# BarnitaSharma/Part-based-3D-Reconstruction

Measured on AMD Instinct MI355X. Metric: Mvoxel/s carved (semantic carve, 1024^3 grid), higher is better.
Workload: dtype u8

## Files before the change

part-based-3d-reconstruction_amd/csrc/ctx.hip:

```cpp
#include <cmath>
#include <cstdlib>

#include <string>

#include "pb3d_internal.h"

static int pool_flush(pb3d_ctx* ctx);

static thread_local char g_err[512] = "";

void pb3d_set_error(const char* fmt, ...) {
    va_list ap;
    va_start(ap, fmt);
    vsnprintf(g_err, sizeof(g_err), fmt, ap);
    va_end(ap);
}

extern "C" {

int pb3d_version(void) { return 101; }

int64_t pb3d_sync_count(pb3d_ctx* ctx) { return ctx ? (int64_t)ctx->sync_count : -1; }

const char* pb3d_last_error(void) { return g_err; }

int pb3d_device_count(int* n) {
    PB3D_REQUIRE(n != nullptr, "pb3d_device_count: null output");
    int c = 0;
    hipError_t e = hipGetDeviceCount(&c);
    if (e != hipSuccess) {
        (void)hipGetLastError();
        c = 0;
    }
    *n = c;
    return PB3D_OK;
}

int pb3d_create(int device, pb3d_ctx** out) {
    PB3D_REQUIRE(out != nullptr, "pb3d_create: null output");
    *out = nullptr;
    int n = 0;
    pb3d_device_count(&n);
    if (n <= 0) {
        pb3d_set_error("pb3d_create: no HIP device visible (libpb3d has no CPU fallback)");
        return PB3D_ENODEVICE;
    }
    PB3D_REQUIRE(device >= 0 && device < n, "pb3d_create: device %d out of range (have %d)", device, n);
    PB3D_HIP(hipSetDevice(device));
    pb3d_ctx* ctx = (pb3d_ctx*)calloc(1, sizeof(pb3d_ctx));
    if (!ctx) {
        pb3d_set_error("pb3d_create: out of host memory");
        return PB3D_ENOMEM;
    }
    ctx->device = device;
    {
        auto env_int = [](const char* name) { const char* v = getenv(name); return v ? atoi(v) : 0; };
        ctx->tune_uncap = env_int("PB3D_UNCAP");
        ctx->tune_sliced = env_int("PB3D_SLICED");
        ctx->tune_s32_gpw = env_int("PB3D_S32_GPW");
        ctx->tune_rot90_wide = env_int("PB3D_ROT90_WIDE");
    }
    hipDeviceProp_t prop;
    hipError_t e = hipGetDeviceProperties(&prop, device);
    if (e != hipSuccess) {
        free(ctx);
        pb3d_set_error("hipGetDeviceProperties failed: %s", hipGetErrorString(e));
        return PB3D_ENODEVICE;
    }
    ctx->cus = prop.multiProcessorCount;
    e = hipStreamCreateWithFlags(&ctx->stream, hipStreamNonBlocking);
    if (e != hipSuccess) {
        free(ctx);
        pb3d_set_error("hipStreamCreate failed: %s", hipGetErrorString(e));
        return PB3D_ENODEVICE;
    }
    e = hipEventCreateWithFlags(&ctx->s32_ev, hipEventDisableTiming);
    if (e != hipSuccess) {
        (void)hipStreamDestroy(ctx->stream);
        free(ctx);
        pb3d_set_error("hipEventCreate failed: %s", hipGetErrorString(e));
        return PB3D_ENODEVICE;
    }
    {
        const char* v = getenv("PB3D_DEVICE_POOL_MB");
        ctx->pool_cap = v ? (size_t)(atoll(v) < 0 ? 0 : atoll(v)) << 20 : (size_t)prop.totalGlobalMem / 4;
    }
    ctx->pinned_bytes = 1 << 16;
    e = hipHostMalloc(&ctx->pinned, ctx->pinned_bytes, hipHostMallocDefault);
    if (e != hipSuccess) {
        (void)hipEventDestroy(ctx->s32_ev);
        (void)hipStreamDestroy(ctx->stream);
        free(ctx);
        pb3d_set_error("hipHostMalloc failed: %s", hipGetErrorString(e));
        return PB3D_ENOMEM;
    }
    if (const char* kn = getenv("PB3D_KNOBS")) {
        std::string all(kn);
        size_t pos = 0;
        while (pos < all.size()) {
            const size_t end = all.find(',', pos);
            const std::string item = all.substr(pos, end == std::string::npos ? std::string::npos : end - pos);
            pos = end == std::string::npos ? all.size() : end + 1;
            if (item.empty()) continue;
            const size_t eq = item.find('=');
            const int rc = eq == std::string::npos ? PB3D_EINVAL : pb3d_set_tuning(ctx, item.substr(0, eq).c_str(), atoi(item.c_str() + eq + 1));
            if (rc != PB3D_OK) {
                if (eq == std::string::npos) pb3d_set_error("PB3D_KNOBS: '%s' is not name=value", item.c_str());
                (void)hipHostFree(ctx->pinned);
                (void)hipEventDestroy(ctx->s32_ev);
                (void)hipStreamDestroy(ctx->stream);
                free(ctx);
                return PB3D_EINVAL;
            }
        }
    }
    *out = ctx;
    return PB3D_OK;
}

namespace {
struct Knob { const char* name; int pb3d_ctx::*field; int lo, hi; const char* what; };
const Knob kKnobs[] = {
    {"sliced", &pb3d_ctx::tune_sliced, 0, 1, "0 (rotation steps on 0/1 data run bit-sliced) or 1 (never: byte chain)"},
    {"rot90_wide", &pb3d_ctx::tune_rot90_wide, 0, 2, "0 (choose), 1 or 2 (the 128-tile / 128-byte-segment kernels)"},
    {"rot90_fill", &pb3d_ctx::tune_rot90_fill, 0, 64, "a count of workgroups per CU (0 = the built-in rule)"},
    {"rot90_order", &pb3d_ctx::tune_rot90_order, 0, 1, "0 (a plane chunk per XCD) or 1 (plain x-fastest order)"},
    {"rot90_flat", &pb3d_ctx::tune_rot90_flat, 0, 2, "0 (choose), 1 (row-wise tile kernel) or 2 (flat on whole-line streams only)"},
    {"rot90_mask_block", &pb3d_ctx::tune_rot90_mask_block, 0, 1, "0 (mask bytes once into LDS) or 1 (per plane / segment)"},
    {"s32_gpw", &pb3d_ctx::tune_s32_gpw, 0, 1 << 20, "a count of plane groups"},
    {"s32_order", &pb3d_ctx::tune_s32_order, 0, 1, "0 (plane groups fastest) or 1 (x fastest)"},
    {"s32_fuse_last", &pb3d_ctx::tune_s32_fuse_last, 0, 1, "0 (fused) or 1 (table step)"},
    {"ccl_blocks", &pb3d_ctx::tune_ccl_blocks, 0, 1 << 20, "a count of workgroups per CU"},
    {"ccl_init_blocks", &pb3d_ctx::tune_ccl_init_blocks, 0, 1 << 20, "a count of workgroups per CU"},
    {"ccl_tilecols", &pb3d_ctx::tune_ccl_tilecols, 0, 64, "at most 64"},
    {"ccl_merge", &pb3d_ctx::tune_ccl_merge, 0, 1, "0 (tile kernels) or 1 (pairwise kernel)"},
    {"orient_tile", &pb3d_ctx::tune_orient_tile, 0, 1, "0 (128-pixel tiles where they apply) or 1 (never)"},
    {"global_composed", &pb3d_ctx::tune_global_composed, 0, 1, "0 (mask bits -> sliced chain -> colours) or 1 (ones -> process -> colour)"},
    {"per_job", &pb3d_ctx::tune_per_job, 0, 1, "0 (merged / fused forms) or 1 (job by job)"},
    {"no_table_cache", &pb3d_ctx::tune_no_table_cache, 0, 1, "0 (tables cached across calls) or 1 (rebuilt every call)"},
    {"part90_inflight", &pb3d_ctx::tune_part90_inflight, 0, 44, "10 UA + UE with UA, UE in 1, 2, 4 (0 = the default 2 / 4)"},
    {"crop_ablate", &pb3d_ctx::tune_crop_ablate, 0, 1 << 20, "ablation switches of k_crop_chain"},
    {"uncap", &pb3d_ctx::tune_uncap, 0, 1, "0 or 1 (every grid-stride kernel as one workgroup per tile)"},
};
}

int pb3d_set_tuning(pb3d_ctx* ctx, const char* name, int value) {
    PB3D_REQUIRE(ctx != nullptr && name != nullptr, "pb3d_set_tuning: null argument");
    for (const Knob& k : kKnobs)
        if (!strcmp(name, k.name)) {
            PB3D_REQUIRE(value >= k.lo && value <= k.hi, "pb3d_set_tuning: %s is %s (got %d)", k.name, k.what, value);
            ctx->*k.field = value;
            return PB3D_OK;
        }
    pb3d_set_error("pb3d_set_tuning: unknown knob '%s'", name);
    return PB3D_EINVAL;
}

int pb3d_make_current(pb3d_ctx* ctx) {
    PB3D_REQUIRE(ctx != nullptr, "pb3d_make_current: null context");
    PB3D_HIP(hipSetDevice(ctx->device));
    return PB3D_OK;
}

void pb3d_destroy(pb3d_ctx* ctx) {
    if (!ctx) return;
    (void)hipSetDevice(ctx->device);
    (void)hipStreamSynchronize(ctx->stream);
    pb3d_comm_destroy(ctx);
    (void)pool_flush(ctx);
    for (int i = 0; i < PB3D_SLOT_COUNT; ++i)
        if (ctx->scratch[i]) (void)hipFree(ctx->scratch[i]);
    if (ctx->pinned) (void)hipHostFree(ctx->pinned);
    if (ctx->stage) (void)hipHostFree(ctx->stage);
    (void)hipEventDestroy(ctx->s32_ev);
    (void)hipStreamDestroy(ctx->stream);
    free(ctx);
}

int pb3d_device_info(pb3d_ctx* ctx, char* name, int name_cap, int* compute_units, int64_t* hbm_bytes) {
    PB3D_REQUIRE(ctx != nullptr, "pb3d_device_info: null context");
    hipDeviceProp_t prop;
    PB3D_HIP(hipGetDeviceProperties(&prop, ctx->device));
    if (name && name_cap > 0) {
        snprintf(name, (size_t)name_cap, "%s (%s)", prop.name, prop.gcnArchName);
    }
    if (compute_units) *compute_units = prop.multiProcessorCount;
    if (hbm_bytes) *hbm_bytes = (int64_t)prop.totalGlobalMem;
    return PB3D_OK;
}

int pb3d_sync(pb3d_ctx* ctx) {
    PB3D_REQUIRE(ctx != nullptr, "pb3d_sync: null context");
    return pb3d_stream_sync(ctx);
}

static int pool_flush(pb3d_ctx* ctx) {
    if (ctx->pool_nfree == 0) return PB3D_OK;
    PB3D_HIP(hipStreamSynchronize(ctx->stream));
    for (int i = 0; i < ctx->pool_nfree; ++i) (void)hipFree(ctx->pool_free[i].p);
    ctx->pool_nfree = 0;
    ctx->pool_cached = 0;
    return PB3D_OK;
}

static hipError_t pool_malloc(pb3d_ctx* ctx, void** p, size_t bytes) {
    hipError_t e = hipMalloc(p, bytes);
    if (e == hipErrorOutOfMemory && ctx->pool_nfree > 0) {
        (void)hipGetLastError();
        if (pool_flush(ctx) == PB3D_OK) e = hipMalloc(p, bytes);
    }
    return e;
}

int pb3d_dev_alloc(pb3d_ctx* ctx, size_t bytes, void** dptr) {
    PB3D_REQUIRE(ctx != nullptr && dptr != nullptr, "pb3d_dev_alloc: null argument");
    *dptr = nullptr;
    PB3D_HIP(hipSetDevice(ctx->device));
    size_t padded = ((bytes ? bytes : 1) + 64 + 255) & ~(size_t)255;
    int best = -1;
    for (int i = 0; i < ctx->pool_nfree; ++i) {
        const size_t b = ctx->pool_free[i].bytes;
        if (b >= padded && b <= padded + padded / 8 + (1u << 20) && (best < 0 || b < ctx->pool_free[best].bytes)) best = i;
    }
    void* p = nullptr;
    size_t got = padded;
    if (best >= 0) {
        p = ctx->pool_free[best].p; got = ctx->pool_free[best].bytes;
        ctx->pool_cached -= got;
        ctx->pool_free[best] = ctx->pool_free[--ctx->pool_nfree];
    } else {
        PB3D_HIP(pool_malloc(ctx, &p, padded));
    }
    if (ctx->pool_cap > 0) {
        if (ctx->pool_nlive < PB3D_POOL_LIVE) ctx->pool_live[ctx->pool_nlive++] = {p, got, 0};
    }
    *dptr = p;
    return PB3D_OK;
}

int pb3d_dev_free(pb3d_ctx* ctx, void* dptr) {
    PB3D_REQUIRE(ctx != nullptr, "pb3d_dev_free: null context");
    if (!dptr) return PB3D_OK;
    size_t bytes = 0;
    for (int i = ctx->pool_nlive - 1; i >= 0; --i)
        if (ctx->pool_live[i].p == dptr) { bytes = ctx->pool_live[i].bytes; ctx->pool_live[i] = ctx->pool_live[--ctx->pool_nlive]; break; }
    if (bytes > 0 && bytes <= ctx->pool_cap) {
        while (ctx->pool_nfree > 0 && (ctx->pool_cached + bytes > ctx->pool_cap || ctx->pool_nfree == PB3D_POOL_SLOTS)) {
            int old = 0;
            for (int i = 1; i < ctx->pool_nfree; ++i)
                if (ctx->pool_free[i].stamp < ctx->pool_free[old].stamp) old = i;
            PB3D_TRY(pb3d_stream_sync(ctx));
            PB3D_HIP(hipFree(ctx->pool_free[old].p));
            ctx->pool_cached -= ctx->pool_free[old].bytes;
            ctx->pool_free[old] = ctx->pool_free[--ctx->pool_nfree];
        }
        ctx->pool_free[ctx->pool_nfree++] = {dptr, bytes, ++ctx->pool_stamp};
        ctx->pool_cached += bytes;
        return PB3D_OK;
    }
    PB3D_TRY(pb3d_stream_sync(ctx));
    PB3D_HIP(hipFree(dptr));
    return PB3D_OK;
}

int pb3d_dev_memset(pb3d_ctx* ctx, void* dptr, int value, size_t bytes) {
    PB3D_REQUIRE(ctx != nullptr && (dptr != nullptr || bytes == 0), "pb3d_dev_memset: null argument");
    if (bytes) PB3D_HIP(hipMemsetAsync(dptr, value, bytes, ctx->stream));
    return PB3D_OK;
}

int pb3d_h2d(pb3d_ctx* ctx, void* dptr, const void* hptr, size_t bytes) {
    PB3D_REQUIRE(ctx != nullptr, "pb3d_h2d: null context");
    if (!bytes) return PB3D_OK;
    PB3D_REQUIRE(dptr && hptr, "pb3d_h2d: null buffer");
    PB3D_HIP(hipMemcpyAsync(dptr, hptr, bytes, hipMemcpyHostToDevice, ctx->stream));
    return pb3d_stream_sync(ctx);
}

int pb3d_h2d_async(pb3d_ctx* ctx, void* dptr, const void* hptr, size_t bytes) {
    PB3D_REQUIRE(ctx != nullptr, "pb3d_h2d_async: null context");
    if (!bytes) return PB3D_OK;
    PB3D_REQUIRE(dptr && hptr, "pb3d_h2d_async: null buffer");
    if (!ctx->stage) {
// ... 137 lines not shown
```

part-based-3d-reconstruction_amd/csrc/pb3d_internal.h:

```cpp
#pragma once
#include <hip/hip_runtime.h>

#include <cstdarg>
#include <cstdint>
#include <cstdio>
#include <cstring>
#include <initializer_list>
#include <type_traits>

#include "pb3d.h"

typedef uint8_t u8;
typedef int64_t i64;
typedef uint64_t u64;
typedef uint32_t u32;

enum pb3d_slot : int {
    PB3D_SLOT_HOST_IN0 = 0,
    PB3D_SLOT_HOST_OUT0 = 1,
    PB3D_SLOT_HOST_IN1 = 2,
    PB3D_SLOT_HOST_OUT1 = PB3D_SLOT_HOST_IN1,
    PB3D_SLOT_HOST_IN2 = 3,
    PB3D_SLOT_HOST_OUT2 = PB3D_SLOT_HOST_IN2,
    PB3D_SLOT_HOST_TMP = PB3D_SLOT_HOST_IN2,
// ... 10 lines not shown
    PB3D_SLOT_RECOLOR_FLAGS = PB3D_SLOT_VOL_TMP,
    PB3D_SLOT_SELECT_FLAGS = PB3D_SLOT_VOL_KEEP,
    PB3D_SLOT_MESH_HOST_COLS = PB3D_SLOT_VOL_OCC,
    PB3D_SLOT_BLOCK_COUNTS = 8,
    PB3D_SLOT_SCAN_LOCAL = 11,
    PB3D_SLOT_SCAN_SEGS = 15,
    PB3D_SLOT_PROJ_WINNER = PB3D_SLOT_BLOCK_COUNTS,
    PB3D_SLOT_DEFORM_ACC = PB3D_SLOT_SCAN_LOCAL,
    PB3D_SLOT_POINTS_OFFSETS = 9,
    PB3D_SLOT_POINTS_MASKS = 25,
    PB3D_SLOT_EXTRACT_OFFSETS = 24,
    PB3D_SLOT_EXTRACT_MASKS = 26,
    PB3D_SLOT_DEFORM_MARKS = 12,
    PB3D_SLOT_DEFORM_BATCH_MARKS = PB3D_SLOT_DEFORM_MARKS,
    PB3D_SLOT_DEFORM_PTS = 13,
    PB3D_SLOT_DEFORM_COLS = 14,
    PB3D_SLOT_PROJ_BATCH_CAMS = 20,
    PB3D_SLOT_PROJ_BATCH_COUNTS = 21,
    PB3D_SLOT_PROJ_BATCH_COLORS = 22,
    PB3D_SLOT_DEFORM_BATCH_TUPLES = PB3D_SLOT_PROJ_BATCH_CAMS,
    PB3D_SLOT_DEFORM_BATCH_COUNTS = PB3D_SLOT_PROJ_BATCH_COUNTS,
    PB3D_SLOT_MEMBERS_COUNTS = 16,
    PB3D_SLOT_MEMBERS_OFFSETS = 17,
    PB3D_SLOT_LABEL_FLAG = 23,
    PB3D_SLOT_NN_REF_COUNTS = 18,
    PB3D_SLOT_NN_REF_STARTS = 19,
    PB3D_SLOT_NN_REF_COORDS = 27,
    PB3D_SLOT_NN_QUERY_COUNTS = 28,
    PB3D_SLOT_NN_QUERY_STARTS = 29,
    PB3D_SLOT_NN_ORDER = 30,
    PB3D_SLOT_NN_SCAN_LOCAL = 31,
    PB3D_SLOT_NN_SCAN_SEGS = 33,
    PB3D_SLOT_NN_BOUNDS_PARTIALS = 41,
    PB3D_SLOT_NN_BOUNDS = 47,
    PB3D_SLOT_VIOU_BITS = 44,
    PB3D_SLOT_VIOU_DILATED = 45,
    PB3D_SLOT_ROT_VALID_TABLE = 10,
    PB3D_SLOT_PART90_JOBS_T = 46,
    PB3D_SLOT_S32_TILE_PROGRAMS = 32,
    PB3D_SLOT_SLICED_FLAG = 34,
    PB3D_SLOT_SLICED_MASK_BITS = 35,
    PB3D_SLOT_GUIDED_DESCS = 36,
    PB3D_SLOT_GUIDED_MASKS = 37,
    PB3D_SLOT_GUIDED_TABLES = 38,
    PB3D_SLOT_GUIDED_COUNTS = 39,
    PB3D_SLOT_GUIDED_SLICES = 43,
    PB3D_SLOT_CCL_RECORDS = 40,
    PB3D_SLOT_CCL_MEMBER_BITS = 42,
    PB3D_SLOT_MESH_BITS = 48,
    PB3D_SLOT_MESH_VERT_OFFSETS = 51,
    PB3D_SLOT_MESH_FACE_OFFSETS = 52,
    PB3D_SLOT_MESH_VERT_COUNTS = 49,
    PB3D_SLOT_MESH_FACE_COUNTS = 50,
    PB3D_SLOT_MESH_VSCAN_LOCAL = 53,
    PB3D_SLOT_MESH_VSCAN_SEGS = 54,
    PB3D_SLOT_MESH_FSCAN_LOCAL = 55,
    PB3D_SLOT_MESH_FSCAN_SEGS = 56,
    PB3D_SLOT_MESH_VERT_BASE = 57,
    PB3D_SLOT_IOU_COUNTS = 58,
    PB3D_SLOT_KNN_REF_IDS = 59,
    PB3D_SLOT_SURF_FLAG = 60,
    PB3D_SLOT_SURF_FACE_NORMALS = 61,
    PB3D_SLOT_SURF_VERT_COUNTS = 62,
    PB3D_SLOT_SURF_VERT_STARTS = 63,
    PB3D_SLOT_SURF_INCIDENT = 64,
    PB3D_SLOT_SURF_SCAN_LOCAL = 65,
    PB3D_SLOT_SURF_SCAN_SEGS = 66,
    PB3D_SLOT_DENSITY_BOUNDS = 67,
    PB3D_SLOT_DENSITY_COUNTS = 68,
    PB3D_SLOT_DENSITY_WEIGHTS = 69,
    PB3D_SLOT_ICP_INDEX_STARTS = 70,
    PB3D_SLOT_ICP_INDEX_COORDS = 71,
    PB3D_SLOT_ICP_INDEX_IDS = 72,
    PB3D_SLOT_ICP_MOVED = 73,
    PB3D_SLOT_ICP_NEAREST = 74,
    PB3D_SLOT_ICP_PARTIALS = 75,
    PB3D_SLOT_PLANE_PARTIALS = 76,
    PB3D_SLOT_CROP_COUNTS = 77,
    PB3D_SLOT_CROP_OFFSETS = 78,
    PB3D_SLOT_CROP_SCAN_LOCAL = 79,
    PB3D_SLOT_CROP_SCAN_SEGS = 80,
    PB3D_SLOT_SELECT = 81,
    PB3D_SLOT_ICP_KEYS = 82,

    PB3D_SLOT_COUNT = 83
};

struct pb3d_nn_grid {
    double lo[3], hi[3];
    double inv[3], h[3];
    int n[3];
    i64 ncells;
};
struct pb3d_nn_index {
    pb3d_nn_grid g;
    i64 nr;
    const i64* starts;
    const double* xs;
    const int* ids;
};
constexpr i64 pb3d_max_points = (1ll << 31) - 1;
template <bool F64>
__device__ __forceinline__ void pb3d_load3(const void* p, i64 i, double* x, double* y, double* z) {
    if (F64) {
        const double* d = (const double*)p + 3 * i;
        *x = d[0]; *y = d[1]; *z = d[2];
    } else {
        const float* f = (const float*)p + 3 * i;
        *x = (double)f[0]; *y = (double)f[1]; *z = (double)f[2];
    }
}
template <bool F64>
__device__ __forceinline__ void pb3d_load3(const void* p, i64 i, double v[3]) { pb3d_load3<F64>(p, i, &v[0], &v[1], &v[2]); }

struct pb3d_pair {
    bool valid;
    int nslots;
    pb3d_slot slot[3];
    u64 use[3];
};

#define PB3D_POOL_SLOTS 64
#define PB3D_POOL_LIVE 4096

struct pb3d_event {
    hipEvent_t ev;
};

struct pb3d_ctx {
    int device;
    int cus;
    hipStream_t stream;
    bool orient_lds_set;
    bool guided_lds_set;
    int tune_rot90_fill;
    int tune_rot90_order;
    int tune_rot90_flat;
    int tune_rot90_mask_block;
    int tune_orient_tile;
    int tune_global_composed;
    int tune_per_job;
    int tune_no_table_cache;
    int tune_part90_inflight;
    int tune_crop_ablate;
    int tune_uncap;
    int tune_sliced;
    int tune_rot90_wide;
    bool rot90w_lds_set;
    bool part90_lds_set;
    bool rot90wf_lds_set;
    int tune_s32_order;
    int tune_s32_fuse_last;
    int tune_s32_gpw;
    int tune_ccl_blocks;
    int tune_ccl_init_blocks;
    int tune_ccl_tilecols;
    int tune_ccl_merge;
    void* scratch[PB3D_SLOT_COUNT];
    size_t scratch_bytes[PB3D_SLOT_COUNT];
    void* pinned;
    size_t pinned_bytes;
    void* stage;
    size_t stage_bytes, stage_head;
    u64 sync_count;
    struct PointsArgs { const void* grid; i64 A0, A1, A2, n, C, ncolors, stride; u8 colors[3 * 32]; };
    struct { pb3d_pair pair; PointsArgs a; } pts_dev, pts;
    struct MeshArgs { const void* grid; i64 A0, A1, A2, nv, nf, C, stride; };
    struct { pb3d_pair pair; MeshArgs a; } mesh_dev, mesh;
    struct { pb3d_pair pair; int ox, oy, oz; i64 X, Y, Z, n; } deform;
    struct ValidCache { void* buf; u64 gen; i64 W, D; double p[8]; } valid_cache;
    struct S32Cache { bool valid; u64 gen; i64 W, D; int ns; double p[32 * 8]; } s32_cache;
    hipEvent_t s32_ev;
    struct CclLast { bool valid; const void* labels; const void* bits; i64 rows, A2, P; u64 gen; bool members_only; int K, C; u32 colors[PB3D_CCL_MAX_COLORS]; } ccl_last;
    struct IcpIndex { bool valid; const void* tgt; i64 nt; int f64; u64 gen[3]; pb3d_nn_index ix; } icp_index;
    struct PoolBlock { void* p; size_t bytes; u64 stamp; };
    PoolBlock pool_free[PB3D_POOL_SLOTS];
    int pool_nfree;
    PoolBlock pool_live[PB3D_POOL_LIVE];
    int pool_nlive;
    size_t pool_cached, pool_cap;
    u64 pool_stamp;
    u64 scratch_gen;
    u64 scratch_slot_gen[PB3D_SLOT_COUNT];
    u64 scratch_use[PB3D_SLOT_COUNT];
    void* rccl_lib;
    void* rccl_comm;
    int rank, nranks;
};

void pb3d_set_error(const char* fmt, ...);

#define PB3D_HIP(call)                                                                          \
    do {                                                                                        \
        hipError_t e_ = (call);                                                                 \
        if (e_ != hipSuccess) {                                                                 \
            pb3d_set_error("%s failed: %s (%s:%d)", #call, hipGetErrorString(e_), __FILE__, __LINE__); \
            return e_ == hipErrorOutOfMemory ? PB3D_ENOMEM : PB3D_ENODEVICE;                    \
        }                                                                                       \
    } while (0)

#define PB3D_TRY(call)                 \
    do {                               \
        int rc_ = (call);              \
        if (rc_ != PB3D_OK) return rc_; \
    } while (0)

#define PB3D_REQUIRE(cond, ...)         \
    do {                                \
        if (!(cond)) {                  \
            pb3d_set_error(__VA_ARGS__); \
            return PB3D_EINVAL;         \
        }                               \
    } while (0)

#define PB3D_CHECK_LAUNCH() PB3D_HIP(hipGetLastError())

int pb3d_scratch(pb3d_ctx* ctx, pb3d_slot slot, size_t bytes, void** out);

void pb3d_pair_record(pb3d_ctx* ctx, pb3d_pair* pr, std::initializer_list<pb3d_slot> slots);
int pb3d_pair_check(const pb3d_ctx* ctx, const pb3d_pair& pr, bool same_args, const char* fill, const char* count);
template <class Args>
bool pb3d_same_args(const Args& a, const Args& b) {
    static_assert(std::has_unique_object_representations_v<Args>, "an argument record compared byte for byte must have no padding");
    return memcmp(&a, &b, sizeof(Args)) == 0;
}
static inline pb3d_ctx::PointsArgs pb3d_points_args(const void* grid, i64 A0, i64 A1, i64 A2, int C, const u8* colors, int ncolors,
                                                    int stride, i64 n) {
    pb3d_ctx::PointsArgs a{grid, A0, A1, A2, n, C, ncolors, stride, {}};
    if (ncolors) memcpy(a.colors, colors, (size_t)(C == 1 ? 1 : 3) * ncolors);
    return a;
}
int pb3d_stream_sync(pb3d_ctx* ctx);

static inline unsigned pb3d_stream_blocks(const pb3d_ctx* ctx, i64 work_items, int per_block, int blocks_per_cu) {
    i64 need = (work_items + per_block - 1) / per_block;
    i64 cap = (blocks_per_cu > 0 && !ctx->tune_uncap) ? (i64)(ctx->cus > 0 ? ctx->cus : 256) * blocks_per_cu : 0x7fffffffll;
    if (need < 1) need = 1;
    return (unsigned)(need < cap ? need : cap);
}

static inline unsigned pb3d_batch_blocks(const pb3d_ctx* ctx, i64 work_items, int per_block, i64 batch, int blocks_per_cu) {
    i64 need = (work_items + per_block - 1) / per_block;
    const i64 cap = ((i64)ctx->cus * blocks_per_cu + batch - 1) / batch;
    if (need > cap) need = cap;
    return (unsigned)(need < 1 ? 1 : need);
}

struct pb3d_magic { u32 m; int sa, sb; u32 d; };
static inline pb3d_magic pb3d_make_magic(u32 d) {
    int L = 0;
    while ((1ull << L) < d) ++L;
    pb3d_magic g;
    g.m = (u32)(((1ull << 32) * ((1ull << L) - d)) / d + 1);
    g.sa = L < 1 ? L : 1;
    g.sb = L > 1 ? L - 1 : 0;
    g.d = d;
    return g;
}
__device__ __forceinline__ u32 pb3d_div(u32 n, const pb3d_magic g) {
    const u32 t = __umulhi(g.m, n);
    return (t + ((n - t) >> g.sa)) >> g.sb;
}

struct pb3d_ccl_dev { const i64* total; const char* records; int dcap; };
int pb3d_ccl_label_on_device(pb3d_ctx* ctx, const uint8_t* d_grid, int64_t A0, int64_t A1, int64_t A2, const uint8_t color[3], int channels, int32_t* d_labels,
                             int64_t cap, pb3d_ccl_dev* dev, int connectivity = 6);

int pb3d_scan_counts(pb3d_ctx* ctx, const u32* d_counts, i64 n, i64* d_offsets, pb3d_slot local_slot, pb3d_slot seg_slot);
int pb3d_nn_index_build(pb3d_ctx* ctx, const void* d_r, int r_f64, i64 nr, pb3d_slot starts_slot, pb3d_slot coords_slot, pb3d_slot ids_slot,
                        pb3d_nn_index* ix);
int pb3d_nn_index_nearest(pb3d_ctx* ctx, const pb3d_nn_index& ix, const double* d_q, i64 nq, int* d_idx);
int pb3d_select_kth(pb3d_ctx* ctx, const double* d_vals, i64 n, const i64* d_rank, double* d_out);
int pb3d_process_grid_sliced(pb3d_ctx* ctx, const u8* d_occ, i64 W, i64 H, i64 D, const u8* d_mask_wh, int angle_interval, u8* d_out,
                             int known_binary, int* took);
int pb3d_global_carve_sliced(pb3d_ctx* ctx, const u8* d_mask_wh, const u8* d_rgb_hw3, i64 W, i64 H, i64 D, int angle_interval, u8* d_out_rgb,
                             int* took);
int pb3d_process_grid_binary_dev(pb3d_ctx* ctx, const u8* d_occ, i64 W, i64 H, i64 D, const u8* d_mask_wh, int angle_interval, u8* d_out,
                                 u8* d_tmp);
int pb3d_rotate_step_sliced(pb3d_ctx* ctx, const u8* d_occ, i64 W, i64 H, i64 D, const double M[9], const double off[3], const u8* d_mask_wh, u8* d_out,
                            int* took);
int pb3d_launch_rotate_generic(pb3d_ctx* ctx, const u8* d_in, i64 W, i64 H, i64 D, const double M[9],
                               const double off[3], const u8* d_mask_wh, u8* d_out, const u8* d_mask_src);
bool pb3d_is_perm_step(const double M[9], const double off[3], i64 W, i64 D);
int pb3d_perm_valid_table(pb3d_ctx* ctx, const double M[9], const double off[3], i64 W, i64 D, u32** bits, int* nw, int* c0, int* c2, bool* rot90);
bool pb3d_perm_step_ok(const double M[9], const double off[3], i64 W, i64 D, const void* a, const void* b);
int pb3d_launch_rotate_perm(pb3d_ctx* ctx, const u8* d_in, i64 W, i64 H, i64 D, const double M[9], const double off[3],
                            const u8* d_mask_src, const u8* d_mask_dst, u8* d_out);
int pb3d_try_part_carve90(pb3d_ctx* ctx, const u8* d_colored, int C, i64 W, i64 H, i64 D, const u8* d_mask_sub, const u8* d_mask_carve,
                          const int* job_angle, const int* job_skip, int njobs, u8* d_out);
int pb3d_transpose_mask_dev(pb3d_ctx* ctx, const u8* d_hw, i64 h, i64 w, u8* d_wh);
int pb3d_part_carve90_planes(pb3d_ctx* ctx, const u8* d_colored, int C, i64 W, i64 H, i64 D, const u32* d_A, const u32* d_AT, int njobs, const u32* d_vbits,
                             int nwv, int c0, int c2, u8* d_out, int* took);
int pb3d_launch_gc90_stream(pb3d_ctx* ctx, const u8* d_bin_hw, const u8* d_rgb_hw3, int C, const u32* d_vbits, int nw, int c0, i64 W, i64 H, i64 D, i64 x0,
                            i64 x1, u8* d_out_slab);
int pb3d_launch_global_carve90(pb3d_ctx* ctx, const u8* d_bin_hw, const u8* d_rgb_hw3, int C, i64 h, i64 w, const double M[9],
                               const double off[3], i64 x0, i64 x1, u8* d_out_slab);
```

part-based-3d-reconstruction_amd/csrc/sliced.hip:

```cpp
#include "rot_common.h"

namespace {

typedef u32 u32x4 __attribute__((ext_vector_type(4)));
typedef u32 u32x2 __attribute__((ext_vector_type(2)));
typedef u32x2 u32x2_a1 __attribute__((aligned(1)));

constexpr int ST = 64;
constexpr int STHREADS = 256;
constexpr int SROWS = 96;
#ifndef PB3D_SPITCH
#define PB3D_SPITCH 101
#endif
constexpr int SPITCH = PB3D_SPITCH;
constexpr int SMAXU = 9;
constexpr int SMAXSTEPS = 32;

struct STile {
    int bx0, bz0, nrows, nunits, fits, pad0, pad1, pad2;
    u32 ugoff[SMAXU * STHREADS];
    unsigned short uloff[SMAXU * STHREADS];
    u32 cellw[16 * STHREADS];
};
static_assert(sizeof(STile) % 16 == 0, "STile is read with 16-byte loads");
// ... 275 lines not shown
        const int idx = tid + 256 * k, r = idx >> 3, cg = idx & 7;
        u32* dst = tile + r * UPITCH + 4 * cg;
        dst[0] = dq[k].x; dst[1] = dq[k].y; dst[2] = dq[k].z; dst[3] = dq[k].w;
    }
    __syncthreads();
    const int zp = tid & 7, xl = tid >> 3;
    const i64 x = x0 + xl, z = z0 + 16 * zp;
    const bool rowlive = x < W;
    const bool live = rowlive && z < D;
    const u32 vb = live ? (vbits[x * nw + (z >> 5)] >> (z & 31)) & 0xffffu : 0u;
    const u32 m = rowlive ? mbits[(i64)g * W + x] : 0u;
    const int np = (int)(H - 32 * (i64)g < 32 ? H - 32 * (i64)g : 32);
    u32 v[4][4];
#pragma unroll
    for (int j = 0; j < 4; ++j) {
        u32 a[4];
#pragma unroll
        for (int c = 0; c < 4; ++c) a[c] = ((vb >> (4 * j + c)) & 1u) ? tile[(16 * zp + 4 * j + c) * UPITCH + xl] & m : 0u;
        tr4x4(a[0], a[1], a[2], a[3], v[j]);
    }
    const bool fullrow = z0 + UZ <= D;
    const i64 rowbase = (((i64)(rowlive ? x : 0) * H + 32 * (i64)g) * D + z0) * 3;
    const u8* px = rgb_hw3 + ((32 * (i64)g) * W + (rowlive ? x : 0)) * 3;
    const int grp = (lane & ~7) * 3;
#pragma unroll
    for (int q = 0; q < 32; ++q) {
        if (q >= np) continue;
        u32 o[12];
        {
            const u8* c = px + (i64)q * W * 3;
            const u32 R = c[0], G = c[1], B = c[2];
            const u32 C0 = R | (G << 8) | (B << 16) | (R << 24), C1 = G | (B << 8) | (R << 16) | (G << 24), C2 = B | (R << 8) | (G << 16) | (B << 24);
#pragma unroll
            for (int j = 0; j < 4; ++j) rgb4((v[j][q >> 3] >> (q & 7)) & 0x01010101u, C0, C1, C2, o + 3 * j);
        }
        if (!fullrow) {
            if (live) {
                u8* dp = out + rowbase + (i64)q * D * 3 + 48 * zp;
                for (int bb = 0; bb < 48 && 3 * z + bb < 3 * D; ++bb) dp[bb] = (u8)(o[bb >> 2] >> (8 * (bb & 3)));
            }
            continue;
        }
#pragma unroll
        for (int k = 0; k < 3; ++k) { u32x4 t4; t4.x = o[4 * k]; t4.y = o[4 * k + 1]; t4.z = o[4 * k + 2]; t4.w = o[4 * k + 3]; win[wv][3 * lane + k] = t4; }
#pragma unroll
        for (int k = 0; k < 3; ++k) {
            const int cidx = 8 * k + zp;
            const u32x4 t4 = win[wv][grp + cidx];
            if (rowlive) *(u32x4_a1*)(out + rowbase + (i64)q * D * 3 + 16 * cidx) = t4;
        }
    }
}

__global__ __launch_bounds__(STHREADS) void k_s32_prep(StepParams sp, i64 W, i64 D, i64 Dp, int ntz, STile* __restrict__ tiles) {
    __shared__ int bb[4];
    __shared__ int rmin[SROWS], rmax[SROWS];
    __shared__ int ustart[SROWS + 1];
    __shared__ int rc0[SROWS];
    const int tid = threadIdx.x;
    const RotParams p = sp.p[blockIdx.y];
    const int t = (int)blockIdx.x;
    STile* o = tiles + (i64)blockIdx.y * gridDim.x + t;
    const i64 x0 = (i64)(t / ntz) * ST, z0 = (i64)(t % ntz) * ST;
    if (tid == 0) { bb[0] = 0x7fffffff; bb[1] = -1; bb[2] = 0x7fffffff; bb[3] = -1; }
    if (tid < SROWS) { rmin[tid] = 0x7fffffff; rmax[tid] = -1; }
    __syncthreads();
    const int tz = tid & 15, jr = tid >> 4;
    int s0[16], s2[16];
    u32 lut[16];
    int mn0 = 0x7fffffff, mx0 = -1, mn2 = 0x7fffffff, mx2 = -1;
#pragma unroll
    for (int i = 0; i < 4; ++i)
#pragma unroll
        for (int c = 0; c < 4; ++c) {
            const int k = 4 * i + c;
            const i64 x = x0 + jr + 16 * i, z = z0 + 4 * tz + c;
            s0[k] = -1; s2[k] = 0; lut[k] = 0;
            if (x < W && z < D) {
                const Cell cl = make_cell(p, x, z, W, D);
                if (cl.s0 >= 0) {
                    s0[k] = cl.s0; s2[k] = cl.s2;
                    lut[k] = lut_of(cl) | (cl.wx1 != 0.0 ? 1u << 16 : 0u) | (cl.wz1 != 0.0 ? 1u << 17 : 0u);
                    const int e0 = cl.s0 + (int)((lut[k] >> 16) & 1u), e2 = cl.s2 + (int)((lut[k] >> 17) & 1u);
                    mn0 = min(mn0, cl.s0); mx0 = max(mx0, e0); mn2 = min(mn2, cl.s2); mx2 = max(mx2, e2);
                }
            }
        }
#pragma unroll
    for (int s = 32; s > 0; s >>= 1) {
        mn0 = min(mn0, __shfl_xor(mn0, s)); mx0 = max(mx0, __shfl_xor(mx0, s));
        mn2 = min(mn2, __shfl_xor(mn2, s)); mx2 = max(mx2, __shfl_xor(mx2, s));
    }
    if ((tid & 63) == 0 && mx0 >= 0) { atomicMin(&bb[0], mn0); atomicMax(&bb[1], mx0); atomicMin(&bb[2], mn2); atomicMax(&bb[3], mx2); }
    __syncthreads();
    const int bx0 = bb[0], bx1 = bb[1], bz0 = bb[2] & ~3, bz1 = bb[3];
    const bool any_valid = bx1 >= 0;
    const int nrows = any_valid ? bx1 - bx0 + 1 : 0;
    bool fits = !any_valid || (nrows + 1 <= SROWS && bz1 - bz0 + 2 <= SPITCH);
    if (fits && any_valid) {
#pragma unroll
        for (int k = 0; k < 16; ++k) {
            if (s0[k] < 0) continue;
            const int r = s0[k] - bx0, e2 = s2[k] + (int)((lut[k] >> 17) & 1u);
            atomicMin(&rmin[r], s2[k]); atomicMax(&rmax[r], e2);
            if ((lut[k] >> 16) & 1u) { atomicMin(&rmin[r + 1], s2[k]); atomicMax(&rmax[r + 1], e2); }
        }
    }
    __syncthreads();
    if (tid < 64) {
        int n[2];
#pragma unroll
        for (int h = 0; h < 2; ++h) {
            const int r = tid + 64 * h;
            n[h] = 0;
            if (r < SROWS) {
                rc0[r] = 0;
                if (r < nrows && fits && rmax[r] >= 0) {
                    rc0[r] = (rmin[r] - bz0) >> 2;
                    n[h] = ((rmax[r] - bz0) >> 2) - ((rmin[r] - bz0) >> 2) + 1;
                }
            }
        }
        int inc0 = n[0], inc1 = n[1];
#pragma unroll
        for (int s = 1; s < 64; s <<= 1) {
            const int a = __shfl_up(inc0, s), b2 = __shfl_up(inc1, s);
            if (tid >= s) { inc0 += a; inc1 += b2; }
        }
        const int tot0 = __shfl(inc0, 63);
        ustart[tid] = inc0 - n[0];
        if (tid + 64 <= SROWS) ustart[tid + 64] = tot0 + inc1 - n[1];
    }
    __syncthreads();
    int nunits = (any_valid && fits) ? ustart[SROWS] : 0;
    if (nunits > SMAXU * STHREADS) { fits = false; nunits = 0; }
    if (fits && tid < nrows) {
        const int u0 = ustart[tid], u1 = ustart[tid + 1];
        for (int u = u0; u < u1; ++u) {
            const int cu = rc0[tid] + (u - u0);
            o->ugoff[u] = (u32)(((i64)bx0 + tid) * Dp + bz0 + 4 * cu);
            o->uloff[u] = (unsigned short)(tid * SPITCH + 4 * cu);
        }
    }
#pragma unroll
    for (int k = 0; k < 16; ++k) {
        u32 w = 0;
        if (fits && s0[k] >= 0) w = (lut[k] << 16) | (u32)((s0[k] - bx0) * SPITCH + (s2[k] - bz0));
        o->cellw[k * STHREADS + tid] = w;
    }
    if (tid == 0) { o->bx0 = bx0; o->bz0 = bz0; o->nrows = nrows; o->nunits = nunits; o->fits = fits ? 1 : 0; o->pad0 = o->pad1 = o->pad2 = 0; }
}

__global__ __launch_bounds__(STHREADS, 4) void k_s32_step(const u32* __restrict__ in, u32* __restrict__ out, const u32* __restrict__ mbits,
                                                           const STile* __restrict__ tiles, i64 W, i64 Dp, int G, int ntz, int ntiles, int gpw,
                                                           int nchunks) {
    __shared__ u32 tile[SROWS * SPITCH];
    const int tid = threadIdx.x;
    const int slot = (int)(blockIdx.x >> 3);
    const int t = slot % ntiles;
    const int chunk = (slot / ntiles) * 8 + (int)(blockIdx.x & 7u);
    if (chunk >= nchunks) return;
    const STile* ti = tiles + t;
    const i64 x0 = (i64)(t / ntz) * ST, z0 = (i64)(t % ntz) * ST;
    const int g_beg = chunk * gpw, g_end = g_beg + gpw < G ? g_beg + gpw : G;
    const int nunits = ti->nunits;
    u32 ug[SMAXU], ul[SMAXU];
#pragma unroll
    for (int j = 0; j < SMAXU; ++j) {
        const int u = tid + STHREADS * j;
        ug[j] = 0xffffffffu; ul[j] = 0;
        if (u < nunits) { ug[j] = ti->ugoff[u]; ul[j] = ti->uloff[u]; }
    }
    u32 cw[16];
#pragma unroll
    for (int i = 0; i < 16; ++i) cw[i] = ti->cellw[i * STHREADS + tid];
    const int tz = tid & 15, jr = tid >> 4;
    const i64 zc = z0 + 4 * tz;
    const bool zok = zc < Dp;
    u32x4 v[SMAXU];
    auto load_group = [&](int g) {
        const u32* src = in + (i64)g * W * Dp;
#pragma unroll
        for (int j = 0; j < SMAXU; ++j)
            if (ug[j] != 0xffffffffu) v[j] = *(const u32x4*)(src + ug[j]);
    };
    load_group(g_beg);
    for (int g = g_beg; g < g_end; ++g) {
#pragma unroll
        for (int j = 0; j < SMAXU; ++j)
            if (ug[j] != 0xffffffffu) { u32* d = tile + ul[j]; d[0] = v[j].x; d[1] = v[j].y; d[2] = v[j].z; d[3] = v[j].w; }
        __syncthreads();
        if (g + 1 < g_end) load_group(g + 1);
#pragma unroll
        for (int i = 0; i < 4; ++i) {
            u32 R[4];
#pragma unroll
            for (int c = 0; c < 4; ++c) {
                const u32 w = cw[4 * i + c];
                const u32* tp = tile + (w & 0xffffu);
                R[c] = lut_apply32(w >> 16, tp[0], tp[1], tp[SPITCH], tp[SPITCH + 1]);
            }
            const i64 x = x0 + jr + 16 * i;
            if (x < W && zok) {
                const u32 m = mbits[(i64)g * W + x];
                u32x4 r; r.x = R[0] & m; r.y = R[1] & m; r.z = R[2] & m; r.w = R[3] & m;
                *(u32x4*)(out + ((i64)g * W + x) * Dp + zc) = r;
            }
        }
        __syncthreads();
    }
}

static bool step_fits(const double M[9]) {
    const double ext0 = fabs(M[0]) + fabs(M[2]), ext2 = fabs(M[6]) + fabs(M[8]);
    return ext0 <= 1.4143 && ext2 <= 1.4143;
}

}

static int s32_chain(pb3d_ctx* ctx, const u8* d_occ, i64 W, i64 H, i64 D, const u8* d_mask_wh, int angle_interval, u8* d_out, const u8* d_rgb_hw3,
                     int known_binary, int* took, const double* Mx = nullptr, const double* offx = nullptr) {
    *took = 0;
    const int nrot = Mx ? 1 : 90 / angle_interval;
    if (ctx->tune_sliced == 1 || nrot < 1) return PB3D_OK;
    if (!Mx && nrot == 1 && angle_interval == 90) {
        const i64 sh[3] = {W, H, D};
        double M[9], off[3];
        PB3D_TRY(pb3d_rotinv(90, M));
        PB3D_TRY(pb3d_offset(M, sh, off));
        if (pb3d_is_perm_step(M, off, W, D)) return PB3D_OK;
    }
    const i64 Dp = (D + 15) & ~(i64)15;
    const int G = (int)((H + 31) / 32);
    const i64 nzb = Dp / 16;
    if (W >= 32768 || D >= 32768 || (i64)G * W * nzb >= (1ll << 31) || W * Dp >= (1ll << 31)) return PB3D_OK;
    const i64 shape[3] = {W, H, D};
    StepParams sp;
    const int ntz = (int)((D + ST - 1) / ST), ntx = (int)((W + ST - 1) / ST), ntiles = ntz * ntx;
    void *flagp, *mb;
    PB3D_TRY(pb3d_scratch(ctx, PB3D_SLOT_SLICED_FLAG, 64, &flagp));
    PB3D_TRY(pb3d_scratch(ctx, PB3D_SLOT_SLICED_MASK_BITS, (size_t)G * W * sizeof(u32), &mb));
    int* flag = (int*)flagp;
    const size_t sbytes = (size_t)G * W * Dp * sizeof(u32);
    void *A = nullptr, *B = nullptr;
    PB3D_TRY(pb3d_dev_alloc(ctx, sbytes, &A));
    int rc = pb3d_dev_alloc(ctx, sbytes, &B);
    if (rc != PB3D_OK) { (void)pb3d_dev_free(ctx, A); return rc; }
    auto body = [&]() -> int {
        if (d_mask_wh) {
            hipLaunchKernelGGL(k_s32_maskbits, dim3((unsigned)(((i64)G * W + 255) / 256)), dim3(256), 0, ctx->stream, d_mask_wh, W, H, G, (u32*)mb, flag);
        } else {
            PB3D_HIP(hipMemsetAsync(mb, 0xff, (size_t)G * W * sizeof(u32), ctx->stream));
            PB3D_HIP(hipMemsetAsync(flag, 0, sizeof(int), ctx->stream));
        }
        const u32 total = (u32)((i64)G * W * nzb);
        const pb3d_magic mzb = pb3d_make_magic((u32)nzb), mw = pb3d_make_magic((u32)W), mg = pb3d_make_magic((u32)G);
        const int gfast = ctx->tune_s32_order == 1;
        if (d_occ) {
            const bool nt = W * H * D >= (i64)256 << 20;
#define PB3D_SLICE(WH, NTL) hipLaunchKernelGGL((k_s32_slice<WH, NTL>), dim3((total + 255u) / 256u), dim3(256), 0, ctx->stream, d_occ, (u32*)A, Mx ? (const u32*)nullptr : (const u32*)mb, W, H, D, Dp, mzb, mw, total, flag, mg, gfast)
            if (D % 16 == 0) { if (nt) PB3D_SLICE(true, true); else PB3D_SLICE(true, false); }
            else { if (nt) PB3D_SLICE(false, true); else PB3D_SLICE(false, false); }
#undef PB3D_SLICE
        } else {
            const u32 tq = (u32)((i64)G * W * (Dp / 4));
            hipLaunchKernelGGL(k_s32_fill, dim3((tq + 255u) / 256u), dim3(256), 0, ctx->stream, (u32*)A, (const u32*)mb, D, Dp, pb3d_make_magic((u32)(Dp / 4)), tq);
        }
        PB3D_CHECK_LAUNCH();
        int* hflag = (int*)((char*)ctx->pinned + ctx->pinned_bytes - 64);
        if (!known_binary) {
            PB3D_HIP(hipMemcpyAsync(hflag, flag, sizeof(int), hipMemcpyDeviceToHost, ctx->stream));
            PB3D_HIP(hipEventRecord(ctx->s32_ev, ctx->stream));
        }
        int gpw = ctx->tune_s32_gpw > 0 ? ctx->tune_s32_gpw : 1;
        if (ctx->tune_s32_gpw <= 0)
            while (gpw < G && (i64)ntiles * ((G + gpw - 1) / gpw) > (i64)ctx->cus * 16) ++gpw;
        const int nchunks = (G + gpw - 1) / gpw;
        const i64 nblk = 8ll * ntiles * ((nchunks + 7) / 8);
        PB3D_REQUIRE(nblk < (1ll << 31), "pb3d_process_grid: grid too large");
        u32 *src = (u32*)A, *dst = (u32*)B;
        bool checked = known_binary != 0;
        int nrot_tab = nrot;
        u32* vbits = nullptr;
        int vnw = 0, pc0 = 0, pc2 = 0;
        if (!Mx && nrot * angle_interval == 90 && ctx->tune_s32_fuse_last != 1 && H <= 65535ll * 32) {
            double M[9], off[3];
            PB3D_TRY(pb3d_rotinv(90, M));
            PB3D_TRY(pb3d_offset(M, shape, off));
            bool rot90 = false;
            if (pb3d_is_perm_step(M, off, W, D)) {
                PB3D_TRY(pb3d_perm_valid_table(ctx, M, off, W, D, &vbits, &vnw, &pc0, &pc2, &rot90));
                if (rot90) nrot_tab = nrot - 1; else vbits = nullptr;
            }
        }
        for (int s0 = 0; s0 < nrot_tab; s0 += SMAXSTEPS) {
            const int ns = nrot_tab - s0 < SMAXSTEPS ? nrot_tab - s0 : SMAXSTEPS;
            memset(&sp, 0, sizeof(sp));
            for (int k = 0; k < ns; ++k) {
                double M[9], off[3];
                if (Mx) { memcpy(M, Mx, sizeof(M)); memcpy(off, offx, sizeof(off)); }
                else {
                    PB3D_TRY(pb3d_rotinv((s0 + k + 1) * angle_interval, M));
                    PB3D_TRY(pb3d_offset(M, shape, off));
                }
                if (!step_fits(M)) return PB3D_EUNSUPPORTED;
                sp.p[k] = RotParams{M[0], M[1], M[2], off[0], M[6], M[7], M[8], off[2]};
            }
            void* tp;
            PB3D_TRY(pb3d_scratch(ctx, PB3D_SLOT_S32_TILE_PROGRAMS, (size_t)ns * ntiles * sizeof(STile), &tp));
            pb3d_ctx::S32Cache& sc = ctx->s32_cache;
            const bool hit = ctx->tune_no_table_cache != 1 && sc.valid && sc.gen == ctx->scratch_gen && sc.W == W && sc.D == D && sc.ns == ns &&
                             memcmp(sc.p, sp.p, sizeof(RotParams) * (size_t)ns) == 0;
            if (!hit) {
                sc.valid = false;
                hipLaunchKernelGGL(k_s32_prep, dim3((unsigned)ntiles, (unsigned)ns), dim3(STHREADS), 0, ctx->stream, sp, W, D, Dp, ntz, (STile*)tp);
                PB3D_CHECK_LAUNCH();
                static_assert(sizeof(sc.p) == sizeof(sp.p), "S32Cache holds one StepParams");
                memcpy(sc.p, sp.p, sizeof(sp.p));
                sc.W = W; sc.D = D; sc.ns = ns; sc.gen = ctx->scratch_gen; sc.valid = nrot_tab <= SMAXSTEPS;
            }
            for (int k = 0; k < ns; ++k) {
                hipLaunchKernelGGL(k_s32_step, dim3((unsigned)nblk), dim3(STHREADS), 0, ctx->stream, (const u32*)src, dst, (const u32*)mb,
                                   (const STile*)tp + (i64)k * ntiles, W, Dp, G, ntz, ntiles, gpw, nchunks);
                u32* t2 = src; src = dst; dst = t2;
            }
            PB3D_CHECK_LAUNCH();
        }
        if (vbits && d_rgb_hw3) {
            const int utz = (int)((D + UZ - 1) / UZ), utx = (int)((W + UX - 1) / UX);
            hipLaunchKernelGGL(k_s32_unslice90_rgb, dim3((unsigned)(utz * utx), (unsigned)G), dim3(256), 0, ctx->stream, (const u32*)src, d_out, d_rgb_hw3,
                               (const u32*)mb, (const u32*)vbits, vnw, W, H, D, Dp, pc0, pc2, utz);
        } else if (vbits) {
            const int utz = (int)((D + UZ - 1) / UZ), utx = (int)((W + UX - 1) / UX);
            hipLaunchKernelGGL(k_s32_unslice90, dim3((unsigned)(utz * utx), (unsigned)G), dim3(256), 0, ctx->stream, (const u32*)src, d_out, (const u32*)mb,
                               (const u32*)vbits, vnw, W, H, D, Dp, pc0, pc2, utz);
        } else if (d_rgb_hw3)
            hipLaunchKernelGGL(k_s32_unslice_rgb, dim3((total + 255u) / 256u), dim3(256), 0, ctx->stream, (const u32*)src, d_out, d_rgb_hw3, W, H, D, Dp, mzb, mw,
                               total);
        else
            hipLaunchKernelGGL(k_s32_unslice, dim3((total + 255u) / 256u), dim3(256), 0, ctx->stream, (const u32*)src, d_out, W, H, D, Dp, mzb, mw, total, mg, gfast);
        PB3D_CHECK_LAUNCH();
        if (!checked) {
            PB3D_HIP(hipEventSynchronize(ctx->s32_ev));
            checked = true;
            if (*hflag != 0) return PB3D_EUNSUPPORTED;
        }
        return PB3D_OK;
    };
    rc = body();
    (void)pb3d_dev_free(ctx, A);
    (void)pb3d_dev_free(ctx, B);
    if (rc == PB3D_EUNSUPPORTED) return PB3D_OK;
    if (rc == PB3D_OK) *took = 1;
    return rc;
}

int pb3d_process_grid_sliced(pb3d_ctx* ctx, const u8* d_occ, i64 W, i64 H, i64 D, const u8* d_mask_wh, int angle_interval, u8* d_out,
                             int known_binary, int* took) {
    return s32_chain(ctx, d_occ, W, H, D, d_mask_wh, angle_interval, d_out, nullptr, known_binary, took);
}

int pb3d_global_carve_sliced(pb3d_ctx* ctx, const u8* d_mask_wh, const u8* d_rgb_hw3, i64 W, i64 H, i64 D, int angle_interval, u8* d_out_rgb,
                             int* took) {
    return s32_chain(ctx, nullptr, W, H, D, d_mask_wh, angle_interval, d_out_rgb, d_rgb_hw3, 1, took);
}

int pb3d_rotate_step_sliced(pb3d_ctx* ctx, const u8* d_occ, i64 W, i64 H, i64 D, const double M[9], const double off[3], const u8* d_mask_wh, u8* d_out,
                            int* took) {
    return s32_chain(ctx, d_occ, W, H, D, d_mask_wh, 90, d_out, nullptr, 0, took, M, off);
}
```

Baseline: 1.177 million.

## Walk s32 step tiles with a resident grid balancing tile-group items

Replaces the per-tile/per-chunk launch of the bit-sliced rotation step with a persistent-style walk: the grid is sized to the number of resident workgroups from an occupancy query, and each workgroup processes an even share of (tile, plane-group) items. It moves to the next tile and slab while prefetching that tile's unit offsets, and it preloads mask words along with each group. It also removes branches on invalid units by pointing them at a padding slot in LDS, and it packs the LDS offsets. The aim is better load balance and fewer short-lived workgroups, at the cost of extra registers and more complex indexing. The old walk remains available through a tuning knob.

Result: no change. 1.177 million (-0.1%).

```diff
diff --git a/part-based-3d-reconstruction_amd/csrc/ctx.hip b/part-based-3d-reconstruction_amd/csrc/ctx.hip
--- a/part-based-3d-reconstruction_amd/csrc/ctx.hip
+++ b/part-based-3d-reconstruction_amd/csrc/ctx.hip
@@ -128,7 +128,8 @@
     {"rot90_flat", &pb3d_ctx::tune_rot90_flat, 0, 2, "0 (choose), 1 (row-wise tile kernel) or 2 (flat on whole-line streams only)"},
     {"rot90_mask_block", &pb3d_ctx::tune_rot90_mask_block, 0, 1, "0 (mask bytes once into LDS) or 1 (per plane / segment)"},
     {"s32_gpw", &pb3d_ctx::tune_s32_gpw, 0, 1 << 20, "a count of plane groups"},
-    {"s32_order", &pb3d_ctx::tune_s32_order, 0, 1, "0 (plane groups fastest) or 1 (x fastest)"},
+    {"s32_walk", &pb3d_ctx::tune_s32_walk, 0, 1, "0 (tile-major resident walk) or 1 (one workgroup per tile and chunk of groups)"},
+    {"s32_order",&pb3d_ctx::tune_s32_order, 0, 1, "0 (plane groups fastest) or 1 (x fastest)"},
     {"s32_fuse_last", &pb3d_ctx::tune_s32_fuse_last, 0, 1, "0 (fused) or 1 (table step)"},
     {"ccl_blocks", &pb3d_ctx::tune_ccl_blocks, 0, 1 << 20, "a count of workgroups per CU"},
     {"ccl_init_blocks", &pb3d_ctx::tune_ccl_init_blocks, 0, 1 << 20, "a count of workgroups per CU"},
diff --git a/part-based-3d-reconstruction_amd/csrc/pb3d_internal.h b/part-based-3d-reconstruction_amd/csrc/pb3d_internal.h
--- a/part-based-3d-reconstruction_amd/csrc/pb3d_internal.h
+++ b/part-based-3d-reconstruction_amd/csrc/pb3d_internal.h
@@ -186,6 +186,8 @@
     int tune_s32_order;
     int tune_s32_fuse_last;
     int tune_s32_gpw;
+    int tune_s32_walk;
+    int s32_resident;
     int tune_ccl_blocks;
     int tune_ccl_init_blocks;
     int tune_ccl_tilecols;
diff --git a/part-based-3d-reconstruction_amd/csrc/sliced.hip b/part-based-3d-reconstruction_amd/csrc/sliced.hip
--- a/part-based-3d-reconstruction_amd/csrc/sliced.hip
+++ b/part-based-3d-reconstruction_amd/csrc/sliced.hip
@@ -451,45 +451,72 @@
 }
 
 __global__ __launch_bounds__(STHREADS, 4) void k_s32_step(const u32* __restrict__ in, u32* __restrict__ out, const u32* __restrict__ mbits,
-                                                           const STile* __restrict__ tiles, i64 W, i64 Dp, int G, int ntz, int ntiles, int gpw,
-                                                           int nchunks) {
-    __shared__ u32 tile[SROWS * SPITCH];
+                                                           const STile* __restrict__ tiles, i64 W, i64 Dp, int G, int ntz, int ntiles, int gslab,
+                                                           int npieces, int per, int extra, int by_unit) {
+    __shared__ u32 tile[SROWS * SPITCH + 4];
     const int tid = threadIdx.x;
-    const int slot = (int)(blockIdx.x >> 3);
-    const int t = slot % ntiles;
-    const int chunk = (slot / ntiles) * 8 + (int)(blockIdx.x & 7u);
-    if (chunk >= nchunks) return;
-    const STile* ti = tiles + t;
-    const i64 x0 = (i64)(t / ntz) * ST, z0 = (i64)(t % ntz) * ST;
-    const int g_beg = chunk * gpw, g_end = g_beg + gpw < G ? g_beg + gpw : G;
-    const int nunits = ti->nunits;
-    u32 ug[SMAXU], ul[SMAXU];
-#pragma unroll
-    for (int j = 0; j < SMAXU; ++j) {
-        const int u = tid + STHREADS * j;
-        ug[j] = 0xffffffffu; ul[j] = 0;
-        if (u < nunits) { ug[j] = ti->ugoff[u]; ul[j] = ti->uloff[u]; }
-    }
-    u32 cw[16];
-#pragma unroll
-    for (int i = 0; i < 16; ++i) cw[i] = ti->cellw[i * STHREADS + tid];
+    const int xcd = (int)(blockIdx.x & 7u), rem = npieces & 7;
+    const int piece = xcd * (npieces >> 3) + (xcd < rem ? xcd : rem) + (int)(blockIdx.x >> 3);
+    int t, g, g_lo, g_end, left;
+    if (by_unit) {
+        t = piece % ntiles;
+        g_lo = (piece / ntiles) * gslab; g_end = g_lo + gslab < G ? g_lo + gslab : G;
+        g = g_lo; left = g_end - g_lo;
+    } else {
+        const int i0 = piece * per + (piece < extra ? piece : extra), slab_items = ntiles * gslab;
+        const int s = i0 / slab_items;
+        g_lo = s * gslab; g_end = g_lo + gslab < G ? g_lo + gslab : G;
+        const int r = i0 - s * slab_items, len = g_end - g_lo;
+        t = r / len; g = g_lo + (r - t * len); left = per + (piece < extra ? 1 : 0);
+    }
+    constexpr int SMAXU2 = (SMAXU + 1) / 2;
+    auto load_units = [&](int tt, u32* pug, u32* pul) {
+        const STile* ti = tiles + tt;
+        const int nunits = ti->nunits;
+#pragma unroll
+        for (int j = 0; j < SMAXU2; ++j) pul[j] = 0;
+#pragma unroll
+        for (int j = 0; j < SMAXU; ++j) {
+            const int u = tid + STHREADS * j;
+            const u32 go = ti->ugoff[u], lo = ti->uloff[u];
+            pug[j] = u < nunits ? go : 0u;
+            pul[j >> 1] |= (u < nunits ? lo : (u32)(SROWS * SPITCH)) << (16 * (j & 1));
+        }
+    };
+    u32 ug[SMAXU], ul[SMAXU2], cw[16];
+    u32 nug[SMAXU], nul[SMAXU2];
+    auto load_cells = [&](int tt) {
+#pragma unroll
+        for (int i = 0; i < 16; ++i) cw[i] = tiles[tt].cellw[i * STHREADS + tid];
+    };
+    load_units(t, ug, ul);
+    load_cells(t);
     const int tz = tid & 15, jr = tid >> 4;
-    const i64 zc = z0 + 4 * tz;
-    const bool zok = zc < Dp;
     u32x4 v[SMAXU];
-    auto load_group = [&](int g) {
-        const u32* src = in + (i64)g * W * Dp;
-#pragma unroll
-        for (int j = 0; j < SMAXU; ++j)
-            if (ug[j] != 0xffffffffu) v[j] = *(const u32x4*)(src + ug[j]);
+    u32 mn[4];
+    auto load_group = [&](int gg, int tt) {
+        const i64 xr = (i64)(tt / ntz) * ST + jr;
+#pragma unroll
+        for (int i = 0; i < 4; ++i) { const i64 x = xr + 16 * i; mn[i] = mbits[(i64)gg * W + (x < W ? x : W - 1)]; }
+        const u32* src = in + (i64)gg * W * Dp;
+#pragma unroll
+        for (int j = 0; j < SMAXU; ++j) v[j] = *(const u32x4*)(src + ug[j]);
     };
-    load_group(g_beg);
-    for (int g = g_beg; g < g_end; ++g) {
-#pragma unroll
-        for (int j = 0; j < SMAXU; ++j)
-            if (ug[j] != 0xffffffffu) { u32* d = tile + ul[j]; d[0] = v[j].x; d[1] = v[j].y; d[2] = v[j].z; d[3] = v[j].w; }
+    load_group(g, t);
+    for (;;) {
+        const u32 m[4] = {mn[0], mn[1], mn[2], mn[3]};
+#pragma unroll
+        for (int j = 0; j < SMAXU; ++j) { u32* d = tile + ((ul[j >> 1] >> (16 * (j & 1))) & 0xffffu); d[0] = v[j].x; d[1] = v[j].y; d[2] = v[j].z; d[3] = v[j].w; }
         __syncthreads();
-        if (g + 1 < g_end) load_group(g + 1);
+        const i64 x0 = (i64)(t / ntz) * ST, zc = (i64)(t % ntz) * ST + 4 * tz;
+        const bool zok = zc < Dp;
+        const bool more = left > 1, tile_done = g + 1 == g_end;
+        int nt = t + 1, ng_lo = g_lo, ng_end = g_end;
+        if (more && !tile_done) load_group(g + 1, t);
+        if (more && tile_done) {
+            if (nt == ntiles) { nt = 0; ng_lo = g_end; ng_end = ng_lo + gslab < G ? ng_lo + gslab : G; }
+            load_units(nt, nug, nul);
+        }
 #pragma unroll
         for (int i = 0; i < 4; ++i) {
             u32 R[4];
@@ -501,12 +528,21 @@
             }
             const i64 x = x0 + jr + 16 * i;
             if (x < W && zok) {
-                const u32 m = mbits[(i64)g * W + x];
-                u32x4 r; r.x = R[0] & m; r.y = R[1] & m; r.z = R[2] & m; r.w = R[3] & m;
+                u32x4 r; r.x = R[0] & m[i]; r.y = R[1] & m[i]; r.z = R[2] & m[i]; r.w = R[3] & m[i];
                 *(u32x4*)(out + ((i64)g * W + x) * Dp + zc) = r;
             }
         }
         __syncthreads();
+        if (!more) break;
+        --left;
+        if (!tile_done) { ++g; continue; }
+#pragma unroll
+        for (int j = 0; j < SMAXU; ++j) ug[j] = nug[j];
+#pragma unroll
+        for (int j = 0; j < SMAXU2; ++j) ul[j] = nul[j];
+        t = nt; g_lo = ng_lo; g_end = ng_end; g = g_lo;
+        load_cells(t);
+        load_group(g, t);
     }
 }
 
@@ -571,12 +607,28 @@
             PB3D_HIP(hipMemcpyAsync(hflag, flag, sizeof(int), hipMemcpyDeviceToHost, ctx->stream));
             PB3D_HIP(hipEventRecord(ctx->s32_ev, ctx->stream));
         }
-        int gpw = ctx->tune_s32_gpw > 0 ? ctx->tune_s32_gpw : 1;
-        if (ctx->tune_s32_gpw <= 0)
-            while (gpw < G && (i64)ntiles * ((G + gpw - 1) / gpw) > (i64)ctx->cus * 16) ++gpw;
-        const int nchunks = (G + gpw - 1) / gpw;
-        const i64 nblk = 8ll * ntiles * ((nchunks + 7) / 8);
-        PB3D_REQUIRE(nblk < (1ll << 31), "pb3d_process_grid: grid too large");
+        const i64 items = (i64)ntiles * G;
+        int gslab, by_unit;
+        i64 npieces;
+        if (ctx->tune_s32_walk == 1) {
+            int gpw = ctx->tune_s32_gpw > 0 ? ctx->tune_s32_gpw : 1;
+            if (ctx->tune_s32_gpw <= 0)
+                while (gpw < G && (i64)ntiles * ((G + gpw - 1) / gpw) > (i64)ctx->cus * 16) ++gpw;
+            gslab = gpw < G ? gpw : G; by_unit = 1; npieces = (i64)ntiles * ((G + gslab - 1) / gslab);
+        } else {
+            if (ctx->s32_resident == 0) {
+                int per_cu = 0;
+                PB3D_HIP(hipOccupancyMaxActiveBlocksPerMultiprocessor(&per_cu, k_s32_step, STHREADS, 0));
+                PB3D_REQUIRE(per_cu > 0, "pb3d_process_grid: k_s32_step does not fit a compute unit");
+                const int r = (per_cu * ctx->cus) & ~7;
+                ctx->s32_resident = r > 8 ? r : 8;
+            }
+            const i64 R = ctx->s32_resident;
+            const i64 gpw = ctx->tune_s32_gpw > 0 ? (i64)ctx->tune_s32_gpw : (items + R - 1) / R;
+            gslab = (int)(gpw < G ? gpw : G); by_unit = 0;
+            npieces = ctx->tune_s32_gpw > 0 ? (items + gpw - 1) / gpw : (items < R ? items : R);
+        }
+        PB3D_REQUIRE(npieces < (1ll << 31), "pb3d_process_grid: grid too large");
         u32 *src = (u32*)A, *dst = (u32*)B;
         bool checked = known_binary != 0;
         int nrot_tab = nrot;
@@ -619,8 +671,9 @@
                 sc.W = W; sc.D = D; sc.ns = ns; sc.gen = ctx->scratch_gen; sc.valid = nrot_tab <= SMAXSTEPS;
             }
             for (int k = 0; k < ns; ++k) {
-                hipLaunchKernelGGL(k_s32_step, dim3((unsigned)nblk), dim3(STHREADS), 0, ctx->stream, (const u32*)src, dst, (const u32*)mb,
-                                   (const STile*)tp + (i64)k * ntiles, W, Dp, G, ntz, ntiles, gpw, nchunks);
+                hipLaunchKernelGGL(k_s32_step, dim3((unsigned)npieces), dim3(STHREADS), 0, ctx->stream, (const u32*)src, dst, (const u32*)mb,
+                                   (const STile*)tp + (i64)k * ntiles, W, Dp, G, ntz, ntiles, gslab, (int)npieces,
+                                   (int)(items / npieces), (int)(items % npieces), by_unit);
                 u32* t2 = src; src = dst; dst = t2;
             }
             PB3D_CHECK_LAUNCH();
```
